# C0ldstudy/PointSecGuard

Measured on AMD Instinct MI355X. Metric: attacked rooms/sec (4096 pts, 40 PGD iters), higher is better.
Workload: dtype f32; 1 GPU; NB non-targeted PGD (eps=0.05, alpha=2/255, 40 iters) on PointNet++ SSG sem_seg, batch=8 rooms x 4096 pts x 9 ch per GPU (BASELINE configs[1]); steps_coalesced_per_launch_max=8, device_batch_rooms=64, launches_in_flight_per_gpu=3, weights=tests/golden/pn2_weights.npz (fitted fixture)

## Files before the change

include/psg.h:

```cpp
#ifndef PSG_H
#define PSG_H

#include <stdint.h>

#ifdef __cplusplus
extern "C" {
#endif

#define PSG_OK 0
#define PSG_ERR_ARG (-1)
#define PSG_ERR_HIP (-2)
#define PSG_ERR_STATE (-3)

typedef struct psg_ctx psg_ctx;
typedef struct psg_pn2_model psg_pn2_model;
typedef struct psg_pn2_ws psg_pn2_ws;
typedef void *psg_stream;

const char *psg_last_error(void);
const char *psg_version(void);
int psg_env_switches(char *buf, int cap);
int psg_diag_build(void);

int psg_ctx_create(int device, psg_ctx **out);
// ... 46 lines not shown
int psg_pn2_forward(psg_pn2_model *model, psg_pn2_ws *ws, int forward, const float *x0, float *logp_out,
                    float *l4_out, psg_stream stream);

int psg_pn2_backward(psg_pn2_model *model, psg_pn2_ws *ws, int forward, const float *dlogp, float *dx0_out,
                     psg_stream stream);
int psg_pn2_backward_full(psg_pn2_model *model, psg_pn2_ws *ws, int forward, const float *dlogp, float *dx0_out,
                          psg_stream stream);

int psg_pn2_forward_lean(psg_pn2_model *model, psg_pn2_ws *ws, int forward, const float *x0, float *logp_out,
                         psg_stream stream);
int psg_pn2_backward_colour(psg_pn2_model *model, psg_pn2_ws *ws, int forward, const float *dlogp, float *dx0_out,
                            psg_stream stream);
int psg_pn2_backward_colour_pgd(psg_pn2_model *model, psg_pn2_ws *ws, int forward, const float *dlogp, float *x,
                                const float *ori, const uint8_t *mask, float alpha, float eps, float dir, int last,
                                psg_stream stream);

const float *psg_pn2_activation_ptr(const psg_pn2_ws *ws, int which);
int psg_pn2_activation_channels(const psg_pn2_ws *ws, int which);


int psg_group_rows(const float *xyz, const float *feat, const float *new_xyz, const int32_t *gidx, int B, int N, int S,
                   int K, int D, int feat_first, float *rows_out, psg_stream stream);
int psg_group_rows_bwd(const float *drows, const int32_t *gidx, int B, int N, int S, int K, int D, int feat_first,
                       float *dfeat, psg_stream stream);
int psg_pw_mlp_fwd(const float *in, int ld_in, int rows, int K, const float *w, const float *bias, int relu, int M,
                   float *out, int ld_out, uint32_t *mask_out, const float *scale, const float *shift, psg_stream stream);
int psg_pw_mlp_bwd(const float *dout, int ld_dout, int rows, int M, const float *wT, const uint32_t *mask_below, int K,
                   float *din, int ld_din, psg_stream stream);
int psg_apply_relu_bits(float *g, int ld, const uint32_t *bits, const float *scale, int rows, int M, psg_stream stream);
int psg_sa_mlp_max_fwd(const float *rows_in, int n_groups, int K, int cin, int n_layers, const int *widths,
// ... 570 lines not shown
```

pointsecguard_amd/_lib.py:

```python
import ctypes
import os

_HERE = os.path.dirname(os.path.abspath(__file__))
LIB_PATH = os.environ.get("PSG_LIBRARY_OVERRIDE") or os.path.join(_HERE, "libpsg.so")

c_f = ctypes.POINTER(ctypes.c_float)
c_i = ctypes.POINTER(ctypes.c_int32)
c_u8 = ctypes.POINTER(ctypes.c_uint8)
c_ll = ctypes.POINTER(ctypes.c_longlong)
vp = ctypes.c_void_p
ci = ctypes.c_int
cf = ctypes.c_float

SIGNATURES = {
    "psg_last_error": (ctypes.c_char_p, []),
    "psg_version": (ctypes.c_char_p, []),
    "psg_env_switches": (ci, [ctypes.c_char_p, ci]),
    "psg_diag_build": (ci, []),
    "psg_ctx_create": (ci, [ci, ctypes.POINTER(vp)]),
    "psg_ctx_destroy": (ci, [vp]),
    "psg_square_distance": (ci, [vp, vp, vp, ci, ci, ci, vp, vp]),
    "psg_fps": (ci, [vp, vp, ci, ci, ci, ci, vp, vp, vp]),
    "psg_gather_points": (ci, [vp, vp, ci, ci, ci, ci, vp, ci, vp, vp]),
    "psg_ball_query": (ci, [vp, vp, ci, vp, ci, ci, ci, cf, ci, vp, vp]),
# ... 20 lines not shown
    "psg_pn2_ws_create": (ci, [vp, ci, ci, ci, ctypes.POINTER(vp)]),
    "psg_pn2_ws_create_arch": (ci, [vp, ci, ci, ci, ci, ctypes.POINTER(vp)]),
    "psg_pn2_ws_destroy": (ci, [vp]),
    "psg_pn2_ws_bytes": (ctypes.c_size_t, [vp]),
    "psg_pn2_debug_read": (ci, [vp, ctypes.POINTER(ctypes.c_ulonglong), ci]),
    "psg_pn2_prof_enable": (ci, [vp, ci]),
    "psg_pn2_prof_read": (ci, [vp, ci, ctypes.POINTER(ctypes.c_double), ctypes.POINTER(ctypes.c_int)]),
    "psg_pn2_plan_build": (ci, [vp, vp, vp, ci, vp]),
    "psg_pn2_plan_ptr": (vp, [vp, ci, ci, ci, ci]),
    "psg_pn2_forward": (ci, [vp, vp, ci, vp, vp, vp, vp]),
    "psg_pn2_backward": (ci, [vp, vp, ci, vp, vp, vp]),
    "psg_pn2_backward_full": (ci, [vp, vp, ci, vp, vp, vp]),
    "psg_pn2_forward_lean": (ci, [vp, vp, ci, vp, vp, vp]),
    "psg_pn2_backward_colour": (ci, [vp, vp, ci, vp, vp, vp]),
    "psg_pn2_backward_colour_pgd": (ci, [vp, vp, ci, vp, vp, vp, vp, cf, cf, cf, ci, vp]),
    "psg_pn2_activation_ptr": (vp, [vp, ci]),
    "psg_pn2_activation_channels": (ci, [vp, ci]),
    "psg_to_point_major": (ci, [vp, ci, ci, ci, vp, vp]),
    "psg_to_channel_major": (ci, [vp, ci, ci, ci, vp, vp]),
    "psg_ce_logp_grad": (ci, [vp, vp, ci, ci, ci, ci, cf, vp, vp, vp]),
    "psg_pgd_step": (ci, [vp, vp, vp, vp, ci, ci, cf, cf, cf, ci, vp]),
    "psg_pgd_step_field": (ci, [vp, vp, vp, vp, ci, ci, ci, cf, cf, cf, ci, vp]),
    "psg_pn2_nb_attack": (ci, [vp, vp, vp, vp, vp, vp, cf, cf, ci, ci, ci, vp, vp]),
    "psg_pointnet_model_create": (ci, [vp, ctypes.POINTER(vp), ctypes.POINTER(vp), ctypes.POINTER(vp)]),
    "psg_pointnet_model_destroy": (ci, [vp]),
    "psg_pointnet_ws_create": (ci, [vp, ci, ci, ctypes.POINTER(vp)]),
    "psg_pointnet_ws_destroy": (ci, [vp]),
    "psg_pointnet_forward": (ci, [vp, vp, vp, vp, vp, vp, vp, vp, vp]),
    "psg_pointnet_backward": (ci, [vp, vp, vp, vp, vp, vp]),
    "psg_pointnet_nb_attack": (ci, [vp, vp, vp, vp, vp, cf, cf, ci, ci, ci, vp, vp]),
# ... 259 lines not shown
```

pointsecguard_amd/csrc/psg_api.hip:

```cpp
#include <mutex>
#include <atomic>
#include <stdarg.h>
#include <stdlib.h>
#include <string.h>
#include <unordered_set>

#include "psg_common.h"

namespace {
thread_local char g_err[512] = "";
}

namespace psg {
struct EnvSwitch { const char *name; char kind; };
static const EnvSwitch kEnvSwitches[] = {
    {"PSG_TRACE_SYNC", 'd'},       {"PSG_GCN_KNN_STATS", 'd'},   {"PSG_KNN_XCD_ORDER", 'p'},  {"PSG_KNN_FINE_CUT_KK", 'p'},  {"PSG_KNN_SAMPLE2_KK", 'p'},  {"PSG_KNN_F32_SAMPLED_KK", 'p'},
    {"PSG_FP1_WAVE", 'p'},         {"PSG_RLA_NO_FUSE16", 'p'},   {"PSG_RLA_ATOMICS", 'p'},    {"PSG_RLA_NO_SPLIT", 'p'},
    {"PSG_RLA_NO_GRAPH", 'p'},     {"PSG_GEMM_SMALL_BELOW", 'p'}, {"PSG_GCN_KNN", 'p'},        {"PSG_GCN_KNN_BF_MAXD", 'p'},
    {"PSG_GCN_PQ_FUSION", 'p'},    {"PSG_GCN_NO_GRAPH", 'p'},    {"PSG_GCN_EDGE_BWD", 'p'},   {"PSG_BALL_QUERY", 'p'},
    {"PSG_PN2_SPLIT", 'p'},          {"PSG_RLA_NO_DIRECT", 'p'},   {"PSG_NU_NO_GRAPH", 'p'},      {"PSG_PN2_GRAPH", 'p'},
    {"PSG_PN2_FPSPLIT", 'p'},        {"PSG_FPS_CFG", 'p'},         {"PSG_PN2_L1T_COLOUR", 'p'},
    {"PSG_PN2_PGD_FUSE", 'p'},       {"PSG_PN2_POOLT_SPARSE", 'p'}, {"PSG_PN2_PW_SIZED", 'p'},
    {"PSG_PN2_BALL_TABLE", 'p'},     {"PSG_PN2_PACK", 'p'},          {"PSG_PN2_PACK_BWD", 'p'},
    {"PSG_PN2_POOLT_ORDER", 'p'},    {"PSG_THREE_NN", 'p'},
#ifdef PSG_DIAG_BUILD
    {"PSG_DIAG", 'r'},
#endif
};

hipError_t copy_sync(void *dst, const void *src, size_t bytes, hipMemcpyKind kind)
{
    if (bytes == 0) return hipSuccess;
    hipStream_t st = nullptr;
    hipError_t e = hipStreamCreateWithFlags(&st, hipStreamNonBlocking);
    if (e != hipSuccess) return e;
    e = hipMemcpyAsync(dst, src, bytes, kind, st);
    if (e == hipSuccess) e = hipStreamSynchronize(st);
    (void)hipStreamDestroy(st);
    return e;
// ... 185 lines not shown
```

pointsecguard_amd/csrc/psg_attack.hip:

```cpp
#include <string.h>

#include "psg_adam.cuh"
#include "psg_common.h"

namespace {

__global__ void to_point_major_kernel(const float *__restrict__ src, float *__restrict__ dst, int C, int N, size_t total)
{
    for (size_t t = (size_t)blockIdx.x * blockDim.x + threadIdx.x; t < total; t += (size_t)gridDim.x * blockDim.x) {
        size_t b = t / N, n = t % N;
        for (int c = 0; c < C; ++c) dst[t * C + c] = src[(b * C + c) * N + n];
    }
}

__global__ void to_channel_major_kernel(const float *__restrict__ src, float *__restrict__ dst, int C, int N,
                                        size_t total)
{
    for (size_t t = (size_t)blockIdx.x * blockDim.x + threadIdx.x; t < total; t += (size_t)gridDim.x * blockDim.x) {
        size_t b = t / N, n = t % N;
        for (int c = 0; c < C; ++c) dst[(b * C + c) * N + n] = src[t * C + c];
    }
}

constexpr int MAXC = 32;

__global__ __launch_bounds__(256) void ce_logp_grad_kernel(const float *__restrict__ logp, const int32_t *__restrict__ labels, int target,
                                                            int rows, int rows_active, int n_cls, float scale, float *__restrict__ dlogp,
                                                            float *__restrict__ cost)
{
    __shared__ float s_z[256 * MAXC];
    const int r0 = blockIdx.x * 256, nr = min(256, rows - r0);
    const float *src = logp + (size_t)r0 * n_cls;
    for (int i = threadIdx.x; i < nr * n_cls; i += 256) s_z[i] = src[i];
    __syncthreads();
    const int r = r0 + (int)threadIdx.x;
    float g[MAXC];
    if ((int)threadIdx.x < nr) {
        if (r >= rows_active) {
            for (int c = 0; c < n_cls; ++c) g[c] = 0.0f;
        } else {
            const float *lp = s_z + threadIdx.x * n_cls;
            float z[MAXC];
            float m = -INFINITY;
            for (int c = 0; c < n_cls; ++c) { z[c] = lp[c]; m = fmaxf(m, z[c]); }
            float s = 0.0f;
            for (int c = 0; c < n_cls; ++c) s += expf(z[c] - m);
            const float lse = logf(s);
            const int y = labels ? labels[r] : target;
            for (int c = 0; c < n_cls; ++c) {
                float lp2 = (z[c] - m) - lse;
                float p = expf(lp2);
                g[c] = (p - (c == y ? 1.0f : 0.0f)) * scale;
                if (cost && c == y) atomicAdd(cost, -lp2 * scale);
            }
        }
    }
    __syncthreads();
    if ((int)threadIdx.x < nr) {
        float *o = s_z + threadIdx.x * n_cls;
        for (int c = 0; c < n_cls; ++c) o[c] = g[c];
    }
    __syncthreads();
    float *dst = dlogp + (size_t)r0 * n_cls;
    for (int i = threadIdx.x; i < nr * n_cls; i += 256) dst[i] = s_z[i];
}

__global__ void pgd_step_kernel(float *__restrict__ x, const float *__restrict__ grad, const float *__restrict__ ori,
                                const uint8_t *__restrict__ mask, int N, size_t total, float step, float eps, int last)
{
    for (size_t t = (size_t)blockIdx.x * blockDim.x + threadIdx.x; t < total * 3; t += (size_t)gridDim.x * blockDim.x) {
// ... 1002 lines not shown
```

pointsecguard_amd/csrc/psg_pn2.hip:

```cpp
#include <algorithm>
#include <cstdlib>
#include <cstring>
#include <vector>

#include "psg_common.h"
#include "psg_pn2_kernels.cuh"
#include "psg_chain.cuh"
#include "psg_pn2_geomgrad.cuh"

using namespace psg;

namespace {

constexpr int MAXL = PSG_PN2_MSG_NUM_LAYERS;
constexpr int NCLS = PSG_PN2_NUM_CLASSES;
const int kS[4] = {1024, 256, 64, 16};

static inline int diag_build_bits()
{
#ifdef PSG_DIAG_BUILD
    static const int bits = psg::env_int("PSG_DIAG", 0);
    return bits;
#else
    return 0;
// ... 279 lines not shown
FwdLayer fwd_layer(const PackedLayer &p, bool relu, uint16_t *mask)
{
    FwdLayer f;
    f.w = p.wf; f.bias = p.bias; f.mask = mask; f.k8 = p.k8f(); f.mb = p.mbf(); f.relu = relu ? 1 : 0;
    return f;
}
BwdLayer bwd_layer(const PackedLayer &p, const uint16_t *mask)
{
    BwdLayer f;
    f.w = p.wb; f.mask = mask; f.k8 = p.k8b(); f.mb = p.mbb();
    return f;
}

enum { TAG_SA_FWD = 0, TAG_FP_FWD = 4, TAG_FP_BWD = 8, TAG_SA_BWD = 12, TAG_FPS = 16, TAG_BALL = 17, TAG_NN = 18,
       TAG_GATHER = 19, TAG_CE = 20, TAG_PGD = 21, TAG_ZERO = 22, TAG_PW_FWD = 23, TAG_PW_BWD = 24,
       TAG_GEOM_GREL = 25, TAG_GEOM_WGRAD = 26, TAG_GEOM_GX = 27, TAG_PACK_PLAN = 28, TAG_COUNT = 29 };

template <typename KernelT, typename ArgsT>
int launch_lds(psg_pn2_ws *ws, int tag, const char *site, KernelT kern, dim3 grid, int threads, int blocks8, int blk,
               const ArgsT &args, hipStream_t st)
{
    size_t lds = (size_t)blocks8 * blk * sizeof(float);
    if (lds > 160 * 1024) { set_error("LDS request %zu exceeds 160 KiB", lds); return PSG_ERR_ARG; }
    if (lds > 48 * 1024) PSG_CHECK_HIP(psg::allow_big_lds((const void *)kern));
    EvScope prof(&ws->prof, tag, 0.0, st);
    hipLaunchKernelGGL(kern, grid, dim3(threads), lds, st, args);
    PSG_LAUNCH_CHECK_AT(site);
    return PSG_OK;
}

inline int layer_blocks(int k8, int mb) { return std::max(k8, mb * 4); }
// ... 574 lines not shown
int run_fp_fwd(psg_pn2_model *m, psg_pn2_ws *ws, int fwd, float *logp, hipStream_t st)
{
    if constexpr (FpCfg<LVL>::P2 != FpCfg<LVL>::P)
        if (ws->Nl[LVL] % FpCfg<LVL>::P2 == 0) return run_fp_fwd_p<LVL, FpCfg<LVL>::P2>(m, ws, fwd, logp, st);
    return run_fp_fwd_p<LVL, FpCfg<LVL>::P>(m, ws, fwd, logp, st);
}

template <int LVL>
int run_fp_bwd(psg_pn2_model *m, psg_pn2_ws *ws, int fwd, const float *logp, const float *dlogp, hipStream_t st)
{
    if constexpr (FpCfg<LVL>::P2 != FpCfg<LVL>::P)
        if (ws->Nl[LVL] % FpCfg<LVL>::P2 == 0) return run_fp_bwd_p<LVL, FpCfg<LVL>::P2>(m, ws, fwd, logp, dlogp, st);
    return run_fp_bwd_p<LVL, FpCfg<LVL>::P>(m, ws, fwd, logp, dlogp, st);
}

__global__ void extract_xyz_kernel(const float *__restrict__ x0, float *__restrict__ xyz, size_t rows)
{
    for (size_t t = (size_t)blockIdx.x * blockDim.x + threadIdx.x; t < rows * 3; t += (size_t)gridDim.x * blockDim.x)
        xyz[t] = x0[(t / 3) * 9 + (t % 3)];
}

__global__ void extract_color_kernel(const float *__restrict__ x0, float *__restrict__ ori, size_t rows)
{
    for (size_t t = (size_t)blockIdx.x * blockDim.x + threadIdx.x; t < rows * 3; t += (size_t)gridDim.x * blockDim.x)
        ori[t] = x0[(t / 3) * 9 + 3 + (t % 3)];
}

__global__ void gather_starts_kernel(const int32_t *__restrict__ starts, int32_t *__restrict__ out, int level, int B,
                                     int P)
{
// ... 630 lines not shown
    }
}

extern "C" const float *psg_pn2_activation_ptr(const psg_pn2_ws *ws, int which)
{
    if (!ws || which < 0 || which > 6) return nullptr;
    return ws->act[which];
}

extern "C" int psg_pn2_activation_channels(const psg_pn2_ws *ws, int which)
{
    if (!ws || which < 0 || which > 6) return 0;
    return ws->actC[which];
}

extern "C" int psg_pn2_forward(psg_pn2_model *m, psg_pn2_ws *ws, int fwd, const float *x0, float *logp_out,
                               float *l4_out, psg_stream stream)
{
    PSG_REQUIRE(m && ws && x0 && logp_out, "psg_pn2_forward: null argument");
    PSG_REQUIRE(m->arch == ws->arch, "psg_pn2_forward: model and workspace were created for different architectures");
    PSG_REQUIRE(fwd >= 0 && fwd < ws->planned, "psg_pn2_forward: plan slot %d not built (planned %d)", fwd, ws->planned);
    hipStream_t st = (hipStream_t)stream;
    int rc;
    ws->x0_fwd = x0;
    for (int l = 0; l < 4; ++l) {
        for (int sc = 0; sc < m->arch->ns; ++sc) {
            if (m->split_fwd[l] && (rc = run_pw_fwd(m, ws, l, sc, fwd, st))) return rc;
            if ((rc = run_sa_fwd(m, ws, l, sc, fwd, x0, st))) return rc;
        }
    }
    if ((rc = run_fp_fwd<3>(m, ws, fwd, nullptr, st))) return rc;
    if ((rc = run_fp_fwd<2>(m, ws, fwd, nullptr, st))) return rc;
    if ((rc = run_fp_fwd<1>(m, ws, fwd, nullptr, st))) return rc;
    if ((rc = run_fp_fwd<0>(m, ws, fwd, ws->logp, st))) return rc;
    if (logp_out != ws->logp)
        PSG_CHECK_HIP(hipMemcpyAsync(logp_out, ws->logp, (size_t)ws->B * ws->N * NCLS * 4, hipMemcpyDeviceToDevice, st));
    if (l4_out)
        PSG_CHECK_HIP(hipMemcpyAsync(l4_out, ws->act[3], (size_t)ws->B * 16 * ws->actC[3] * 4, hipMemcpyDeviceToDevice, st));
    ws->fwd_slot = fwd;
    return PSG_OK;
}

static int backward_impl(psg_pn2_model *m, psg_pn2_ws *ws, int fwd, const float *logp, const float *dlogp,
                         float *dx0, int c_lo, int c_hi, hipStream_t st, const PgdFuse *pgd = nullptr, bool rel0 = false)
{
    const ArchDesc &A = *m->arch;
    int rc;
    if ((rc = run_fp_bwd<0>(m, ws, fwd, logp, dlogp, st))) return rc;
    if ((rc = run_fp_bwd<1>(m, ws, fwd, nullptr, nullptr, st))) return rc;
    if ((rc = run_fp_bwd<2>(m, ws, fwd, nullptr, nullptr, st))) return rc;
    if ((rc = run_fp_bwd<3>(m, ws, fwd, nullptr, nullptr, st))) return rc;
    for (int l = 3; l >= 0; --l) {
        for (int sc = 0; sc < A.ns; ++sc) {
            if ((rc = run_sa_bwd(m, ws, l, sc, fwd, l ? 0 : c_lo, l ? A.C[l] : (rel0 ? A.C[0] + 3 : c_hi), st))) return rc;
            if (m->split[l] && (rc = run_pw_bwd(m, ws, l, sc, fwd, st))) return rc;
        }
    }
    {
        EvScope prof(&ws->prof, TAG_ZERO, 0.0, st);
        const bool compact = c_hi - c_lo == 3;
        const size_t total = (size_t)ws->B * ws->N * (compact ? 1 : c_hi - c_lo);
        const dim3 grid((unsigned)std::min<size_t>(8192, (total + 255) / 256));
        const size_t po = (size_t)fwd * ws->B * (ws->N + 1);
// ... 154 lines not shown
}
extern "C" int psg_pn2_backward_colour(psg_pn2_model *m, psg_pn2_ws *ws, int fwd, const float *dlogp, float *dx0_out, psg_stream stream)
{
    return psg::pn2_backward_colour(m, ws, fwd, dlogp, dx0_out, stream);
}
extern "C" int psg_pn2_backward_colour_pgd(psg_pn2_model *m, psg_pn2_ws *ws, int fwd, const float *dlogp, float *x, const float *ori,
                                           const uint8_t *mask, float alpha, float eps, float dir, int last, psg_stream stream)
{
    PSG_REQUIRE(m && ws && dlogp && x && ori, "psg_pn2_backward_colour_pgd: null argument");
    PSG_REQUIRE(dir == 1.0f || dir == -1.0f, "psg_pn2_backward_colour_pgd: dir must be +1 or -1");
    if (int rc = require_resident(m, ws, fwd, "psg_pn2_backward_colour_pgd")) return rc;
    const PgdFuse pf{x, ori, mask, dir * alpha, eps, last ? 1 : 0};
    return backward_impl(m, ws, fwd, ws->logp, dlogp, ws->dx0, 3, 6, (hipStream_t)stream, &pf);
}

extern "C" int psg_pn2_nb_attack(psg_pn2_model *m, psg_pn2_ws *ws, const float *images, const int32_t *labels,
                                 const int32_t *starts, const uint8_t *mask, float eps, float alpha, int iters,
                                 int targeted, int target, float *adv_out, psg_stream stream)
{
    PSG_REQUIRE(m && ws && images && starts && adv_out, "psg_pn2_nb_attack: null argument");
    PSG_REQUIRE(m->arch == ws->arch, "psg_pn2_nb_attack: model and workspace were created for different architectures");
    PSG_REQUIRE(targeted || labels, "psg_pn2_nb_attack: labels required for the non-targeted attack");
    PSG_REQUIRE(iters > 0 && iters <= ws->F, "psg_pn2_nb_attack: iters=%d exceeds workspace capacity %d", iters, ws->F);
    hipStream_t st = (hipStream_t)stream;
    const int B = ws->B, N = ws->N;
    int rc;
    if ((rc = psg_to_point_major(images, B, 9, N, ws->x0, st))) return rc;
    if (!targeted) PSG_CHECK_HIP(hipMemcpyAsync(ws->nb_labels, labels, (size_t)B * N * sizeof(int32_t), hipMemcpyDeviceToDevice, st));
    PSG_CHECK_HIP(hipMemcpyAsync(ws->nb_starts, starts, (size_t)iters * 4 * B * sizeof(int32_t), hipMemcpyDeviceToDevice, st));
    if (mask) PSG_CHECK_HIP(hipMemcpyAsync(ws->nb_mask, mask, (size_t)N, hipMemcpyDeviceToDevice, st));
    const int32_t *labels_ws = targeted ? nullptr : ws->nb_labels;
    const uint8_t *mask_ws = mask ? ws->nb_mask : nullptr;
    auto body = [&](hipStream_t st) -> int {
        int r;
        hipLaunchKernelGGL(extract_color_kernel, dim3(std::min(1024, ceil_div(B * N * 3, 256))), dim3(256), 0, st, ws->x0,
                           ws->ori, (size_t)B * N);
        PSG_LAUNCH_CHECK();
        if ((r = psg_pn2_plan_build(ws, ws->x0, ws->nb_starts, iters, st))) return r;
        const int rows = B * N;
        for (int it = 0; it < iters; ++it) {
            if ((r = psg::pn2_forward_lean(m, ws, it, ws->x0, ws->logp, st))) return r;
            {
                EvScope prof(&ws->prof, TAG_CE, 0.0, st);
                if ((r = psg_ce_logp_grad(ws->logp, labels_ws, target, rows, targeted ? N : rows, NCLS, 1.0f / (float)N, ws->dlogp,
                                          nullptr, st)))
                    return r;
            }
            static const bool pgd_fuse = psg::env_int("PSG_PN2_PGD_FUSE", 1) != 0;
            if (pgd_fuse) {
                const PgdFuse pf{ws->x0, ws->ori, mask_ws, (targeted ? -1.0f : 1.0f) * alpha, eps, it == iters - 1 ? 1 : 0};
                if ((r = backward_impl(m, ws, it, ws->logp, ws->dlogp, ws->dx0, 3, 6, st, &pf))) return r;
            } else {
                if ((r = backward_impl(m, ws, it, ws->logp, ws->dlogp, ws->dx0, 3, 6, st))) return r;
                EvScope prof(&ws->prof, TAG_PGD, 0.0, st);
                if ((r = psg_pgd_step(ws->x0, ws->dx0, ws->ori, mask_ws, B, N, alpha, eps, targeted ? -1.0f : 1.0f, it == iters - 1, st)))
                    return r;
            }
        }
        return PSG_OK;
    };
    static const bool use_graph = psg::env_int("PSG_PN2_GRAPH", 0) != 0 && !psg::trace_sync_enabled();
    if (use_graph && B <= 16 && !ws->prof.on) {
        const psg_pn2_ws::NbKey key{m->gen, eps, alpha, iters, targeted ? 1 : 0, targeted ? target : 0, mask ? 1 : 0, targeted ? 0 : 1, 0};
        const bool same = ws->nb_have_key && memcmp(&key, &ws->nb_key, sizeof(key)) == 0;
        if (same && !ws->nb.capture_failed) {
            if (!ws->nb_stream) {
                PSG_CHECK_HIP(hipStreamCreateWithFlags(&ws->nb_stream, hipStreamNonBlocking));
                for (hipEvent_t &e : ws->nb_ev) PSG_CHECK_HIP(hipEventCreateWithFlags(&e, hipEventDisableTiming));
            }
            hipStream_t gs = ws->nb_stream;
            PSG_CHECK_HIP(hipEventRecord(ws->nb_ev[0], st));
            PSG_CHECK_HIP(hipStreamWaitEvent(gs, ws->nb_ev[0], 0));
            if (ws->nb.exec || ws->nb.capture(gs, [&] { return body(gs); })) {
                PSG_CHECK_HIP(ws->nb.replay(gs));
                ws->planned = iters; ws->fwd_slot = iters - 1; ws->x0_fwd = ws->x0;
                PSG_CHECK_HIP(hipEventRecord(ws->nb_ev[1], gs));
                PSG_CHECK_HIP(hipStreamWaitEvent(st, ws->nb_ev[1], 0));
                return psg_to_channel_major(ws->x0, B, 9, N, adv_out, st);
            }
        }
        if (!same) {
            PSG_CHECK_HIP(ws->nb.forget(st));
            ws->nb_key = key;
            ws->nb_have_key = true;
        }
        ws->nb.note_eager();
    }
    if ((rc = body(st))) return rc;
    return psg_to_channel_major(ws->x0, B, 9, N, adv_out, st);
}
// ... 1 lines not shown
```

pointsecguard_amd/csrc/psg_pn2_kernels.cuh:

```cuda
#pragma once
#include "psg_mlp.cuh"

#ifdef PSG_DIAG_BUILD
#define PSG_DIAGBIT(a, bit) ((a).diag & (bit))
#else
#define PSG_DIAGBIT(a, bit) 0
#endif

namespace psg {

struct SaFwdArgs {
    const float *xyz;
    const float *feat;
    const float *new_xyz;
    const int32_t *gidx;
    float *out;
    uint8_t *arg;
    FwdLayer l1, l2;
    const float4 *w3;
    const float *b3;
    int k8_3, nb3;
    int xyz_stride, D, Np, S, C3;
    int ld_out, c_out;
    const float *tfeat;
// ... 1752 lines not shown
    for (int j = rg; j < P; j += RG) {
        const unsigned o = __umul24((unsigned)j, (unsigned)w2);
        for (int q = ql; q < (w2 >> 2); q += 32) *(float4 *)(d2 + (o + 4u * q)) = *(const float4 *)(in + L::off(o2 + 4 * q, j));
    }
    if (!d1) return;
    if (a.split) {
        layer_bwd<P, NW, MAXT>(a.skipT, in, wg);
        __syncthreads();
    }
    for (int j = rg; j < P; j += RG) {
        const unsigned o = __umul24((unsigned)j, (unsigned)a.C1);
        for (int q = ql; q < (a.C1 >> 2); q += 32) *(float4 *)(d1 + (o + 4u * q)) = *(const float4 *)(in + L::off(4 * q, j));
    }
}

struct PwBwdArgs {
    const int32_t *ginv_off;
    const float *gsa;
    int g_rows;
    const float *skip;
    float *out;
    BwdLayer wt;
    int N, C1, D;
};

template <int P, int NW, int VW>
__device__ __forceinline__ void pw_bwd_gather_rows(const PwBwdArgs &a, int b, int n0, float *__restrict__ buf, int lane, int wave)
{
    static_assert(P == 32, "one 32-point tile per workgroup");
    typedef float vwf __attribute__((ext_vector_type(VW)));
// ... 129 lines not shown
```

pointsecguard_amd/runtime.py:

```python
import ctypes

import numpy as np
import torch

from . import _lib

SA_NPOINT = (1024, 256, 64, 16)
SA_RADIUS = (0.1, 0.2, 0.4, 0.8)
NSAMPLE = 32
SA_PACK_GROUPS = (4, 2, 1, 1)
SA_WIDTH3 = (64, 128, 256, 512)
NUM_CLASSES = 13
ARCH_SSG, ARCH_MSG = 0, 1
ARCH_LAYERS = {ARCH_SSG: 23, ARCH_MSG: 35}
MSG_NSAMPLE = (16, 32)
ACT_POINTS = (1024, 256, 64, 16, 64, 256, 1024)
ACT_SHAPES = ((1024, 64), (256, 128), (64, 256), (16, 512), (64, 256), (256, 256), (1024, 128))

_ctx = {}
_hip = None


def ptr(t):
    if t is None:
# ... 192 lines not shown
        out = torch.empty_like(images)
        _lib.call("psg_to_channel_major", ptr(x0), B, 9, N, ptr(out), stream())
        return out

    def backward_pgd(self, model, slot, dlogp, x0, ori, alpha, eps, mask=None, descent=False, last=False):
        require_cuda(dlogp, "dlogp", torch.float32)
        require_cuda(x0, "x0", torch.float32)
        require_cuda(ori, "ori", torch.float32)
        if mask is not None:
            require_cuda(mask, "mask", torch.uint8)
        assert x0.shape == (self.batch, self.n_point, 9) and ori.shape == (self.batch, self.n_point, 3) and x0.is_contiguous() and ori.is_contiguous()
        _lib.call("psg_pn2_backward_colour_pgd", model.handle, self.handle, slot, ptr(dlogp), ptr(x0), ptr(ori), ptr(mask),
                  float(alpha), float(eps), -1.0 if descent else 1.0, 1 if last else 0, stream())
        return x0

    def nb_attack(self, model, images, labels, starts, eps, alpha, iters, mask=None, target=None, out=None):
        require_cuda(images, "images", torch.float32)
        require_cuda(starts, "starts", torch.int32)
        if labels is not None:
            require_cuda(labels, "labels", torch.int32)
        if mask is not None:
            require_cuda(mask, "mask", torch.uint8)
        if out is None:
            out = torch.empty_like(images)
        _lib.call("psg_pn2_nb_attack", model.handle, self.handle, ptr(images), ptr(labels), ptr(starts), ptr(mask),
                  float(eps), float(alpha), int(iters), 0 if target is None else 1, 0 if target is None else int(target),
                  ptr(out), stream())
        return out

    PROF_TAGS = ("sa1_fwd", "sa2_fwd", "sa3_fwd", "sa4_fwd", "fp1_head_fwd", "fp2_fwd", "fp3_fwd", "fp4_fwd",
                 "fp1_head_bwd", "fp2_bwd", "fp3_bwd", "fp4_bwd", "sa1_bwd", "sa2_bwd", "sa3_bwd", "sa4_bwd",
                 "fps", "ball_query", "three_nn", "gather", "ce_grad", "pgd_step", "dx0_gather", "pw_fwd", "pw_bwd",
                 "geom_grel", "geom_wgrad", "geom_gx", "sa_pack_plan")

    def prof_enable(self, on=True):
        _lib.call("psg_pn2_prof_enable", self.handle, 1 if on else 0)

    def prof_read(self):
        n = len(self.PROF_TAGS)
        ms = (ctypes.c_double * n)()
        cnt = (ctypes.c_int * n)()
        _lib.call("psg_pn2_prof_read", self.handle, n, ms, cnt)
        return {t: (ms[i], cnt[i]) for i, t in enumerate(self.PROF_TAGS) if cnt[i]}

    def plan_tensor(self, what, level, forward, room):
        n_l = (self.n_point,) + SA_NPOINT
        k0 = MSG_NSAMPLE[0] if self.arch == ARCH_MSG else NSAMPLE
        shape, dt = {0: ((SA_NPOINT[level],), torch.int32), 1: ((SA_NPOINT[level], k0), torch.int32),
# ... 448 lines not shown
```

Before: 1042 rooms/s.

## Fuse FP1 head forward, cross-entropy grad and FP1 backward into one kernel

Adds a single fp1_loop_kernel that runs the FP1 layers and classifier head forward, computes log-softmax and the cross-entropy gradient in LDS, then runs the FP1/head backward chain in the same workgroup, writing only the gradient into FP2. The PGD attack loop is refactored into an nb_step that takes this path when the model shape matches, skipping the separate FP1 forward, CE kernel and FP1 backward launches along with their global-memory round trips for activations, logp and dlogp. The CE row math is shared through a new header. The cost is a complex, shape-specialised kernel with heavy LDS and register use, and a gate that falls back to the old path when the layer configuration differs.

```diff
diff --git a/include/psg.h b/include/psg.h
--- a/include/psg.h
+++ b/include/psg.h
@@ -84,6 +84,10 @@
 int psg_pn2_backward_colour_pgd(psg_pn2_model *model, psg_pn2_ws *ws, int forward, const float *dlogp, float *x,
                                 const float *ori, const uint8_t *mask, float alpha, float eps, float dir, int last,
                                 psg_stream stream);
+
+int psg_pn2_nb_step(psg_pn2_model *model, psg_pn2_ws *ws, int forward, float *x, const float *ori, const int32_t *labels,
+                    const uint8_t *mask, float alpha, float eps, int targeted, int target, int last, psg_stream stream);
+const float *psg_pn2_fp1_grad_ptr(const psg_pn2_ws *ws);
 
 const float *psg_pn2_activation_ptr(const psg_pn2_ws *ws, int which);
 int psg_pn2_activation_channels(const psg_pn2_ws *ws, int which);
diff --git a/pointsecguard_amd/_lib.py b/pointsecguard_amd/_lib.py
--- a/pointsecguard_amd/_lib.py
+++ b/pointsecguard_amd/_lib.py
@@ -58,6 +58,8 @@
     "psg_pn2_forward_lean": (ci, [vp, vp, ci, vp, vp, vp]),
     "psg_pn2_backward_colour": (ci, [vp, vp, ci, vp, vp, vp]),
     "psg_pn2_backward_colour_pgd": (ci, [vp, vp, ci, vp, vp, vp, vp, cf, cf, cf, ci, vp]),
+    "psg_pn2_nb_step": (ci, [vp, vp, ci, vp, vp, vp, vp, cf, cf, ci, ci, ci, vp]),
+    "psg_pn2_fp1_grad_ptr": (vp, [vp]),
     "psg_pn2_activation_ptr": (vp, [vp, ci]),
     "psg_pn2_activation_channels": (ci, [vp, ci]),
     "psg_to_point_major": (ci, [vp, ci, ci, ci, vp, vp]),
diff --git a/pointsecguard_amd/csrc/psg_api.hip b/pointsecguard_amd/csrc/psg_api.hip
--- a/pointsecguard_amd/csrc/psg_api.hip
+++ b/pointsecguard_amd/csrc/psg_api.hip
@@ -22,7 +22,7 @@
     {"PSG_PN2_FPSPLIT", 'p'},        {"PSG_FPS_CFG", 'p'},         {"PSG_PN2_L1T_COLOUR", 'p'},
     {"PSG_PN2_PGD_FUSE", 'p'},       {"PSG_PN2_POOLT_SPARSE", 'p'}, {"PSG_PN2_PW_SIZED", 'p'},
     {"PSG_PN2_BALL_TABLE", 'p'},     {"PSG_PN2_PACK", 'p'},          {"PSG_PN2_PACK_BWD", 'p'},
-    {"PSG_PN2_POOLT_ORDER", 'p'},    {"PSG_THREE_NN", 'p'},
+    {"PSG_PN2_POOLT_ORDER", 'p'},    {"PSG_THREE_NN", 'p'},         {"PSG_PN2_FP1_LOOP", 'p'},
 #ifdef PSG_DIAG_BUILD
     {"PSG_DIAG", 'r'},
 #endif
diff --git a/pointsecguard_amd/csrc/psg_attack.hip b/pointsecguard_amd/csrc/psg_attack.hip
--- a/pointsecguard_amd/csrc/psg_attack.hip
+++ b/pointsecguard_amd/csrc/psg_attack.hip
@@ -1,6 +1,7 @@
 #include <string.h>
 
 #include "psg_adam.cuh"
+#include "psg_ce_row.cuh"
 #include "psg_common.h"
 
 namespace {
@@ -22,7 +23,7 @@
     }
 }
 
-constexpr int MAXC = 32;
+constexpr int MAXC = psg::CE_ROW_MAXC;
 
 __global__ __launch_bounds__(256) void ce_logp_grad_kernel(const float *__restrict__ logp, const int32_t *__restrict__ labels, int target,
                                                             int rows, int rows_active, int n_cls, float scale, float *__restrict__ dlogp,
@@ -36,24 +37,10 @@
     const int r = r0 + (int)threadIdx.x;
     float g[MAXC];
     if ((int)threadIdx.x < nr) {
-        if (r >= rows_active) {
-            for (int c = 0; c < n_cls; ++c) g[c] = 0.0f;
-        } else {
-            const float *lp = s_z + threadIdx.x * n_cls;
-            float z[MAXC];
-            float m = -INFINITY;
-            for (int c = 0; c < n_cls; ++c) { z[c] = lp[c]; m = fmaxf(m, z[c]); }
-            float s = 0.0f;
-            for (int c = 0; c < n_cls; ++c) s += expf(z[c] - m);
-            const float lse = logf(s);
-            const int y = labels ? labels[r] : target;
-            for (int c = 0; c < n_cls; ++c) {
-                float lp2 = (z[c] - m) - lse;
-                float p = expf(lp2);
-                g[c] = (p - (c == y ? 1.0f : 0.0f)) * scale;
-                if (cost && c == y) atomicAdd(cost, -lp2 * scale);
-            }
-        }
+        const bool active = r < rows_active;
+        const int y = !active ? -1 : labels ? labels[r] : target;
+        const float term = psg::ce_row_grad(s_z + threadIdx.x * n_cls, n_cls, y, scale, active, g);
+        if (cost && active && y >= 0 && y < n_cls) atomicAdd(cost, term);
     }
     __syncthreads();
     if ((int)threadIdx.x < nr) {
diff --git a/pointsecguard_amd/csrc/psg_ce_row.cuh b/pointsecguard_amd/csrc/psg_ce_row.cuh
--- /dev/null
+++ b/pointsecguard_amd/csrc/psg_ce_row.cuh
@@ -0,0 +1,37 @@
+#pragma once
+#include <math.h>
+
+#if defined(__HIPCC__) || defined(__CUDACC__)
+#define PSG_CE_ROW_FN __host__ __device__ __forceinline__
+#else
+#define PSG_CE_ROW_FN inline
+#endif
+
+namespace psg {
+
+constexpr int CE_ROW_MAXC = 32;
+
+PSG_CE_ROW_FN float ce_row_grad(const float *lp, int n_cls, int y, float scale, bool active, float *g)
+{
+#pragma clang fp contract(off)
+    if (!active) {
+        for (int c = 0; c < n_cls; ++c) g[c] = 0.0f;
+        return 0.0f;
+    }
+    float z[CE_ROW_MAXC];
+    float m = -INFINITY;
+    for (int c = 0; c < n_cls; ++c) { z[c] = lp[c]; m = fmaxf(m, z[c]); }
+    float s = 0.0f;
+    for (int c = 0; c < n_cls; ++c) s += __builtin_expf(z[c] - m);
+    const float lse = __builtin_logf(s);
+    float term = 0.0f;
+    for (int c = 0; c < n_cls; ++c) {
+        const float lp2 = (z[c] - m) - lse;
+        const float p = __builtin_expf(lp2);
+        g[c] = (p - (c == y ? 1.0f : 0.0f)) * scale;
+        if (c == y) term = -lp2 * scale;
+    }
+    return term;
+}
+
+}
diff --git a/pointsecguard_amd/csrc/psg_pn2.hip b/pointsecguard_amd/csrc/psg_pn2.hip
--- a/pointsecguard_amd/csrc/psg_pn2.hip
+++ b/pointsecguard_amd/csrc/psg_pn2.hip
@@ -317,7 +317,8 @@
 
 enum { TAG_SA_FWD = 0, TAG_FP_FWD = 4, TAG_FP_BWD = 8, TAG_SA_BWD = 12, TAG_FPS = 16, TAG_BALL = 17, TAG_NN = 18,
        TAG_GATHER = 19, TAG_CE = 20, TAG_PGD = 21, TAG_ZERO = 22, TAG_PW_FWD = 23, TAG_PW_BWD = 24,
-       TAG_GEOM_GREL = 25, TAG_GEOM_WGRAD = 26, TAG_GEOM_GX = 27, TAG_PACK_PLAN = 28, TAG_COUNT = 29 };
+       TAG_GEOM_GREL = 25, TAG_GEOM_WGRAD = 26, TAG_GEOM_GX = 27, TAG_PACK_PLAN = 28, TAG_FP1_LOOP = 29,
+       TAG_COUNT = 30 };
 
 template <typename KernelT, typename ArgsT>
 int launch_lds(psg_pn2_ws *ws, int tag, const char *site, KernelT kern, dim3 grid, int threads, int blocks8, int blk,
@@ -922,6 +923,57 @@
     return run_fp_bwd_p<LVL, FpCfg<LVL>::P>(m, ws, fwd, logp, dlogp, st);
 }
 
+bool fp1_loop_applies(const psg_pn2_model *m, const psg_pn2_ws *ws)
+{
+    static const bool on = psg::env_int("PSG_PN2_FP1_LOOP", 1) != 0;
+#ifdef PSG_DIAG_BUILD
+    constexpr bool diag_build = true;
+#else
+    constexpr bool diag_build = false;
+#endif
+    if (!on || diag_build || FpCfg<0>::P2 != 64 || FpCfg<0>::NW != 4 || fp1_wave() || !m->fsplit[0] || ws->Nl[0] % 64) return false;
+    const ArchDesc &A = *m->arch;
+    const int first = A.fp_first[0], head = A.head;
+    if (A.fp_count[0] != 3 || NCLS != 13 || m->fa[0].k8f() != 0 || m->fa[0].cout != 128 || m->fb[0].cout != 128) return false;
+    for (const PackedLayer *p : {&m->L[first + 1], &m->L[first + 2], &m->L[head]})
+        if (p->k8f() != 16 || p->mbf() != 4 || p->k8b() != 16 || p->mbb() != 4) return false;
+    const PackedLayer &c2 = m->L[head + 1];
+    return c2.k8f() == 16 && c2.mbf() == 1 && c2.k8b() == 2 && c2.mbb() == 4;
+}
+
+int run_fp1_loop(psg_pn2_model *m, psg_pn2_ws *ws, int fwd, const int32_t *labels, int target, int rows_active, float scale,
+                 hipStream_t st)
+{
+    constexpr int P = 64, NW = 4;
+    const ArchDesc &A = *m->arch;
+    const int B = ws->B, N = ws->Nl[0], first = A.fp_first[0], head = A.head;
+    const size_t prob = (size_t)fwd * B;
+    Fp1LoopArgs a{};
+    a.fwd.nn_idx = ws->nn_idx[0] + prob * N * 3;
+    a.fwd.nn_w = ws->nn_w[0] + prob * N * 3;
+    a.fwd.tsrc = ws->tfp[0]; a.fwd.ldt = m->fa[0].cout;
+    a.fwd.N = N; a.fwd.S = ws->Nl[1];
+    a.fwd.layer[0] = fwd_layer(m->fa[0], true, nullptr);
+    a.fwd.layer[0].bias = m->L[first].bias;
+    a.f[0] = fwd_layer(m->L[first + 1], true, nullptr);
+    a.f[1] = fwd_layer(m->L[first + 2], true, nullptr);
+    a.f[2] = fwd_layer(m->L[head], true, nullptr);
+    a.head = fwd_layer(m->L[head + 1], false, nullptr);
+    a.t[0] = bwd_layer(m->L[head + 1], nullptr);
+    a.t[1] = bwd_layer(m->L[head], nullptr);
+    a.t[2] = bwd_layer(m->L[first + 2], nullptr);
+    a.t[3] = bwd_layer(m->L[first + 1], nullptr);
+    a.labels = labels; a.target = target; a.rows_active = rows_active; a.scale = scale;
+    a.dint_out = ws->dint[0];
+    a.N = N;
+#if PSG_MLP_PAIRS
+    return launch_lds(ws, TAG_FP1_LOOP, PSG_SITE, (fp1_loop_kernel<P, NW, NCLS>), dim3(N / P, B), NW * 64, 16 + PSG_LDS_SPARE, Lds<P>::BLK, a, st);
+#else
+    set_error("run_fp1_loop: built without the paired k-loop");
+    return PSG_ERR_STATE;
+#endif
+}
+
 __global__ void extract_xyz_kernel(const float *__restrict__ x0, float *__restrict__ xyz, size_t rows)
 {
     for (size_t t = (size_t)blockIdx.x * blockDim.x + threadIdx.x; t < rows * 3; t += (size_t)gridDim.x * blockDim.x)
@@ -1582,13 +1634,8 @@
     return ws->actC[which];
 }
 
-extern "C" int psg_pn2_forward(psg_pn2_model *m, psg_pn2_ws *ws, int fwd, const float *x0, float *logp_out,
-                               float *l4_out, psg_stream stream)
-{
-    PSG_REQUIRE(m && ws && x0 && logp_out, "psg_pn2_forward: null argument");
-    PSG_REQUIRE(m->arch == ws->arch, "psg_pn2_forward: model and workspace were created for different architectures");
-    PSG_REQUIRE(fwd >= 0 && fwd < ws->planned, "psg_pn2_forward: plan slot %d not built (planned %d)", fwd, ws->planned);
-    hipStream_t st = (hipStream_t)stream;
+static int forward_to_fp2(psg_pn2_model *m, psg_pn2_ws *ws, int fwd, const float *x0, hipStream_t st)
+{
     int rc;
     ws->x0_fwd = x0;
     for (int l = 0; l < 4; ++l) {
@@ -1599,7 +1646,18 @@
     }
     if ((rc = run_fp_fwd<3>(m, ws, fwd, nullptr, st))) return rc;
     if ((rc = run_fp_fwd<2>(m, ws, fwd, nullptr, st))) return rc;
-    if ((rc = run_fp_fwd<1>(m, ws, fwd, nullptr, st))) return rc;
+    return run_fp_fwd<1>(m, ws, fwd, nullptr, st);
+}
+
+extern "C" int psg_pn2_forward(psg_pn2_model *m, psg_pn2_ws *ws, int fwd, const float *x0, float *logp_out,
+                               float *l4_out, psg_stream stream)
+{
+    PSG_REQUIRE(m && ws && x0 && logp_out, "psg_pn2_forward: null argument");
+    PSG_REQUIRE(m->arch == ws->arch, "psg_pn2_forward: model and workspace were created for different architectures");
+    PSG_REQUIRE(fwd >= 0 && fwd < ws->planned, "psg_pn2_forward: plan slot %d not built (planned %d)", fwd, ws->planned);
+    hipStream_t st = (hipStream_t)stream;
+    int rc;
+    if ((rc = forward_to_fp2(m, ws, fwd, x0, st))) return rc;
     if ((rc = run_fp_fwd<0>(m, ws, fwd, ws->logp, st))) return rc;
     if (logp_out != ws->logp)
         PSG_CHECK_HIP(hipMemcpyAsync(logp_out, ws->logp, (size_t)ws->B * ws->N * NCLS * 4, hipMemcpyDeviceToDevice, st));
@@ -1610,11 +1668,12 @@
 }
 
 static int backward_impl(psg_pn2_model *m, psg_pn2_ws *ws, int fwd, const float *logp, const float *dlogp,
-                         float *dx0, int c_lo, int c_hi, hipStream_t st, const PgdFuse *pgd = nullptr, bool rel0 = false)
+                         float *dx0, int c_lo, int c_hi, hipStream_t st, const PgdFuse *pgd = nullptr, bool rel0 = false,
+                         bool fp1_done = false)
 {
     const ArchDesc &A = *m->arch;
     int rc;
-    if ((rc = run_fp_bwd<0>(m, ws, fwd, logp, dlogp, st))) return rc;
+    if (!fp1_done && (rc = run_fp_bwd<0>(m, ws, fwd, logp, dlogp, st))) return rc;
     if ((rc = run_fp_bwd<1>(m, ws, fwd, nullptr, nullptr, st))) return rc;
     if ((rc = run_fp_bwd<2>(m, ws, fwd, nullptr, nullptr, st))) return rc;
     if ((rc = run_fp_bwd<3>(m, ws, fwd, nullptr, nullptr, st))) return rc;
@@ -1799,6 +1858,53 @@
     return backward_impl(m, ws, fwd, ws->logp, dlogp, ws->dx0, 3, 6, (hipStream_t)stream, &pf);
 }
 
+static int nb_step(psg_pn2_model *m, psg_pn2_ws *ws, int fwd, float *x, const float *ori, const int32_t *labels, const uint8_t *mask,
+                   float alpha, float eps, int targeted, int target, bool last, hipStream_t st)
+{
+    const int B = ws->B, N = ws->N, rows = B * N;
+    const int rows_active = targeted ? N : rows;
+    const float scale = 1.0f / (float)N, dir = targeted ? -1.0f : 1.0f;
+    const bool fused = fp1_loop_applies(m, ws);
+    int r;
+    if (fused) {
+        PSG_REQUIRE(fwd >= 0 && fwd < ws->planned, "psg_pn2_nb_step: plan slot %d not built (planned %d)", fwd, ws->planned);
+        ws->lean = true;
+        r = forward_to_fp2(m, ws, fwd, x, st);
+        ws->lean = false;
+        ws->fwd_slot = -1;
+        if (r) return r;
+        if ((r = run_fp1_loop(m, ws, fwd, labels, target, rows_active, scale, st))) return r;
+    } else {
+        if ((r = psg::pn2_forward_lean(m, ws, fwd, x, ws->logp, st))) return r;
+        EvScope prof(&ws->prof, TAG_CE, 0.0, st);
+        if ((r = psg_ce_logp_grad(ws->logp, labels, target, rows, rows_active, NCLS, scale, ws->dlogp, nullptr, st))) return r;
+    }
+    static const bool pgd_fuse = psg::env_int("PSG_PN2_PGD_FUSE", 1) != 0;
+    if (pgd_fuse) {
+        const PgdFuse pf{x, ori, mask, dir * alpha, eps, last ? 1 : 0};
+        return backward_impl(m, ws, fwd, ws->logp, ws->dlogp, ws->dx0, 3, 6, st, &pf, false, fused);
+    }
+    if ((r = backward_impl(m, ws, fwd, ws->logp, ws->dlogp, ws->dx0, 3, 6, st, nullptr, false, fused))) return r;
+    EvScope prof(&ws->prof, TAG_PGD, 0.0, st);
+    return psg_pgd_step(x, ws->dx0, ori, mask, B, N, alpha, eps, dir, last, st);
+}
+
+extern "C" int psg_pn2_nb_step(psg_pn2_model *m, psg_pn2_ws *ws, int fwd, float *x, const float *ori, const int32_t *labels,
+                               const uint8_t *mask, float alpha, float eps, int targeted, int target, int last, psg_stream stream)
+{
+    PSG_REQUIRE(m && ws && x && ori, "psg_pn2_nb_step: null argument");
+    PSG_REQUIRE(m->arch == ws->arch, "psg_pn2_nb_step: model and workspace were created for different architectures");
+    PSG_REQUIRE(targeted || labels, "psg_pn2_nb_step: labels required for the non-targeted step");
+    PSG_REQUIRE(!targeted || (target >= 0 && target < NCLS), "psg_pn2_nb_step: target class %d out of range", target);
+    PSG_REQUIRE(fwd >= 0 && fwd < ws->planned, "psg_pn2_nb_step: plan slot %d not built (planned %d)", fwd, ws->planned);
+    return nb_step(m, ws, fwd, x, ori, targeted ? nullptr : labels, mask, alpha, eps, targeted, target, last != 0, (hipStream_t)stream);
+}
+
+extern "C" const float *psg_pn2_fp1_grad_ptr(const psg_pn2_ws *ws)
+{
+    return ws ? ws->dint[0] : nullptr;
+}
+
 extern "C" int psg_pn2_nb_attack(psg_pn2_model *m, psg_pn2_ws *ws, const float *images, const int32_t *labels,
                                  const int32_t *starts, const uint8_t *mask, float eps, float alpha, int iters,
                                  int targeted, int target, float *adv_out, psg_stream stream)
@@ -1822,26 +1928,8 @@
                            ws->ori, (size_t)B * N);
         PSG_LAUNCH_CHECK();
         if ((r = psg_pn2_plan_build(ws, ws->x0, ws->nb_starts, iters, st))) return r;
-        const int rows = B * N;
-        for (int it = 0; it < iters; ++it) {
-            if ((r = psg::pn2_forward_lean(m, ws, it, ws->x0, ws->logp, st))) return r;
-            {
-                EvScope prof(&ws->prof, TAG_CE, 0.0, st);
-                if ((r = psg_ce_logp_grad(ws->logp, labels_ws, target, rows, targeted ? N : rows, NCLS, 1.0f / (float)N, ws->dlogp,
-                                          nullptr, st)))
-                    return r;
-            }
-            static const bool pgd_fuse = psg::env_int("PSG_PN2_PGD_FUSE", 1) != 0;
-            if (pgd_fuse) {
-                const PgdFuse pf{ws->x0, ws->ori, mask_ws, (targeted ? -1.0f : 1.0f) * alpha, eps, it == iters - 1 ? 1 : 0};
-                if ((r = backward_impl(m, ws, it, ws->logp, ws->dlogp, ws->dx0, 3, 6, st, &pf))) return r;
-            } else {
-                if ((r = backward_impl(m, ws, it, ws->logp, ws->dlogp, ws->dx0, 3, 6, st))) return r;
-                EvScope prof(&ws->prof, TAG_PGD, 0.0, st);
-                if ((r = psg_pgd_step(ws->x0, ws->dx0, ws->ori, mask_ws, B, N, alpha, eps, targeted ? -1.0f : 1.0f, it == iters - 1, st)))
-                    return r;
-            }
-        }
+        for (int it = 0; it < iters; ++it)
+            if ((r = nb_step(m, ws, it, ws->x0, ws->ori, labels_ws, mask_ws, alpha, eps, targeted, target, it == iters - 1, st))) return r;
         return PSG_OK;
     };
     static const bool use_graph = psg::env_int("PSG_PN2_GRAPH", 0) != 0 && !psg::trace_sync_enabled();
@@ -1858,7 +1946,7 @@
             PSG_CHECK_HIP(hipStreamWaitEvent(gs, ws->nb_ev[0], 0));
             if (ws->nb.exec || ws->nb.capture(gs, [&] { return body(gs); })) {
                 PSG_CHECK_HIP(ws->nb.replay(gs));
-                ws->planned = iters; ws->fwd_slot = iters - 1; ws->x0_fwd = ws->x0;
+                ws->planned = iters; ws->fwd_slot = fp1_loop_applies(m, ws) ? -1 : iters - 1; ws->x0_fwd = ws->x0;
                 PSG_CHECK_HIP(hipEventRecord(ws->nb_ev[1], gs));
                 PSG_CHECK_HIP(hipStreamWaitEvent(st, ws->nb_ev[1], 0));
                 return psg_to_channel_major(ws->x0, B, 9, N, adv_out, st);
diff --git a/pointsecguard_amd/csrc/psg_pn2_kernels.cuh b/pointsecguard_amd/csrc/psg_pn2_kernels.cuh
--- a/pointsecguard_amd/csrc/psg_pn2_kernels.cuh
+++ b/pointsecguard_amd/csrc/psg_pn2_kernels.cuh
@@ -1,4 +1,5 @@
 #pragma once
+#include "psg_ce_row.cuh"
 #include "psg_mlp.cuh"
 
 #ifdef PSG_DIAG_BUILD
@@ -1790,6 +1791,181 @@
     }
 }
 
+struct Fp1LoopArgs {
+    FpFwdArgs fwd;
+    FwdLayer f[3];
+    FwdLayer head;
+    BwdLayer t[4];
+    const int32_t *labels;
+    int target, rows_active;
+    float scale;
+    float *dint_out;
+    int N;
+};
+
+__device__ __forceinline__ void add_bias16(f32x16 &c, const float4 &bq0, const float4 &bq1, const float4 &bq2, const float4 &bq3)
+{
+    c[0] += bq0.x; c[1] += bq0.y; c[2] += bq0.z; c[3] += bq0.w;
+    c[4] += bq1.x; c[5] += bq1.y; c[6] += bq1.z; c[7] += bq1.w;
+    c[8] += bq2.x; c[9] += bq2.y; c[10] += bq2.z; c[11] += bq2.w;
+    c[12] += bq3.x; c[13] += bq3.y; c[14] += bq3.z; c[15] += bq3.w;
+}
+
+template <int P>
+__device__ __forceinline__ unsigned fp1_loop_pair_bits(const float *__restrict__ buf, int first, int lane)
+{
+    const int j = lane & 31, h = lane >> 5;
+    const float *o = buf + (size_t)(first * 4) * Lds<P>::BLK + j * 8 + 4 * h;
+    unsigned m = 0;
+#pragma unroll
+    for (int pb = 0; pb < 2; ++pb) {
+#pragma unroll
+        for (int g = 0; g < 4; ++g) {
+            const float4 v = *(const float4 *)(o + (size_t)g * Lds<P>::BLK + pb * 32 * 8);
+            m |= (v.x > 0.0f ? 1u : 0u) << (16 * pb + 4 * g);
+            m |= (v.y > 0.0f ? 1u : 0u) << (16 * pb + 4 * g + 1);
+            m |= (v.z > 0.0f ? 1u : 0u) << (16 * pb + 4 * g + 2);
+            m |= (v.w > 0.0f ? 1u : 0u) << (16 * pb + 4 * g + 3);
+        }
+    }
+    return m;
+}
+
+template <int P>
+__device__ __forceinline__ unsigned fp1_loop_pair_fwd(const FwdLayer &Lr, float *__restrict__ buf, int first, int lane)
+{
+    constexpr int BLK = Lds<P>::BLK;
+    const int j = lane & 31, h = lane >> 5;
+    const float4 *bp = (const float4 *)(Lr.bias + first * 32 + 4 * h);
+    const float4 bq0 = bp[0], bq1 = bp[2], bq2 = bp[4], bq3 = bp[6];
+    f32x16 c0, c1;
+#pragma unroll
+    for (int r = 0; r < 16; ++r) { c0[r] = 0.0f; c1[r] = 0.0f; }
+    tile_mac_x2<BLK, false>(Lr.w + (size_t)first * Lr.k8 * 64 + lane, Lr.k8, buf + j * 8 + 4 * h, c0, c1);
+    add_bias16(c0, bq0, bq1, bq2, bq3);
+    const unsigned m0 = relu_bits(c0);
+    add_bias16(c1, bq0, bq1, bq2, bq3);
+    const unsigned m1 = relu_bits(c1);
+    __syncthreads();
+    store_tile<P>(buf, first, j, h, c0);
+    store_tile<P>(buf, first, 32 + j, h, c1);
+    return m0 | (m1 << 16);
+}
+
+template <int P>
+__device__ __forceinline__ void fp1_loop_pair_bwd(const BwdLayer &Lt, float *__restrict__ buf, int first, int lane, unsigned m)
+{
+    constexpr int BLK = Lds<P>::BLK;
+    const int j = lane & 31, h = lane >> 5;
+    f32x16 c0, c1;
+#pragma unroll
+    for (int r = 0; r < 16; ++r) { c0[r] = 0.0f; c1[r] = 0.0f; }
+    tile_mac_x2<BLK, false>(Lt.w + (size_t)first * Lt.k8 * 64 + lane, Lt.k8, buf + j * 8 + 4 * h, c0, c1);
+    apply_bits(c0, m);
+    apply_bits(c1, m >> 16);
+    __syncthreads();
+    store_tile<P>(buf, first, j, h, c0);
+    store_tile<P>(buf, first, 32 + j, h, c1);
+}
+
+template <int P, int NW, int NC>
+__global__ __launch_bounds__(NW * 64) __attribute__((amdgpu_waves_per_eu(4))) void fp1_loop_kernel(Fp1LoopArgs a)
+{
+    static_assert(P == 64 && NW == 4 && NC <= 16, "one pair of tiles per wave and 128-wide layer; the classes in two LDS blocks");
+    using L = Lds<P>;
+    constexpr int NT = NW * 64;
+    extern __shared__ float lds[];
+    float *buf0 = lds;
+    const int tid = threadIdx.x, lane = tid & 63, wave = tid >> 6;
+    const int j = lane & 31, h = lane >> 5;
+    int bx, b;
+    xcd_tile(bx, b);
+    const int n0 = bx * P;
+    const size_t wg = (size_t)b * gridDim.x + bx;
+    const int first = (wave + (int)(wg & (NW - 1))) & (NW - 1);
+
+    fp_layer1_split<P, NW>(a.fwd, b, n0, buf0, wg);
+    __syncthreads();
+    const unsigned m_l1 = fp1_loop_pair_bits<P>(buf0, first, lane);
+    const unsigned m_l2 = fp1_loop_pair_fwd<P>(a.f[0], buf0, first, lane);
+    __syncthreads();
+    const unsigned m_l3 = fp1_loop_pair_fwd<P>(a.f[1], buf0, first, lane);
+    __syncthreads();
+    const unsigned m_c1 = fp1_loop_pair_fwd<P>(a.f[2], buf0, first, lane);
+    __syncthreads();
+    {
+        f32x16 c;
+        if (first < P / 32) {
+            const float4 *bp = (const float4 *)(a.head.bias + 4 * h);
+            const float4 bq0 = bp[0], bq1 = bp[2], bq2 = bp[4], bq3 = bp[6];
+#pragma unroll
+            for (int r = 0; r < 16; ++r) c[r] = 0.0f;
+            c = tile_mac<L::BLK, false>(a.head.w + lane, a.head.k8, buf0 + (first * 32 + j) * 8 + 4 * h, c);
+            add_bias16(c, bq0, bq1, bq2, bq3);
+        }
+        __syncthreads();
+        if (first < P / 32) store_tile<P>(buf0, 0, first * 32 + j, h, c);
+    }
+    __syncthreads();
+
+    float *s_lp = buf0 + (size_t)4 * L::BLK, *s_dl = buf0 + (size_t)6 * L::BLK;
+    for (int t = tid; t < P * 8; t += NT) {
+        const int pj = t >> 3, q = t & 7;
+        const bool has0 = q < NC;
+        const float z0 = has0 ? buf0[L::off(q, pj)] : -INFINITY;
+        const bool has1 = q + 8 < NC;
+        const float z1 = has1 ? buf0[L::off(q + 8, pj)] : -INFINITY;
+        float m = fmaxf(z0, z1);
+        m = fmaxf(m, __shfl_xor(m, 1));
+        m = fmaxf(m, __shfl_xor(m, 2));
+        m = fmaxf(m, __shfl_xor(m, 4));
+        float s = (has0 ? expf(z0 - m) : 0.0f) + (has1 ? expf(z1 - m) : 0.0f);
+        s += __shfl_xor(s, 1);
+        s += __shfl_xor(s, 2);
+        s += __shfl_xor(s, 4);
+        const float lse = logf(s);
+        float *o = s_lp + pj * NC;
+        if (has0) o[q] = (z0 - m) - lse;
+        if (has1) o[q + 8] = (z1 - m) - lse;
+    }
+    __syncthreads();
+    if (tid < P) {
+        const int r = b * a.N + n0 + tid;
+        const bool active = r < a.rows_active;
+        const int y = !active ? -1 : a.labels ? a.labels[r] : a.target;
+        ce_row_grad(s_lp + tid * NC, NC, y, a.scale, active, s_dl + tid * NC);
+    }
+    __syncthreads();
+    for (int t = tid; t < P * 4; t += NT) {
+        const int pj = t >> 2, q = t & 3;
+        const float *lp = s_lp + pj * NC, *dl = s_dl + pj * NC;
+        float s = 0.0f;
+        if (q == 0)
+            for (int c = 0; c < NC; ++c) s += dl[c];
+        s = __shfl(s, (tid & 63) & ~3);
+#pragma unroll
+        for (int i = 0; i < 4; ++i) {
+            const int c = q + 4 * i;
+            buf0[L::off(c, pj)] = c < NC ? dl[c] - expf(lp[c]) * s : 0.0f;
+        }
+    }
+    __syncthreads();
+
+    fp1_loop_pair_bwd<P>(a.t[0], buf0, first, lane, m_c1);
+    __syncthreads();
+    fp1_loop_pair_bwd<P>(a.t[1], buf0, first, lane, m_l3);
+    __syncthreads();
+    fp1_loop_pair_bwd<P>(a.t[2], buf0, first, lane, m_l2);
+    __syncthreads();
+    fp1_loop_pair_bwd<P>(a.t[3], buf0, first, lane, m_l1);
+    __syncthreads();
+    constexpr int RG = NT / 32, CD = 128;
+    const int ql = tid & 31, rg = tid >> 5;
+    float *d2 = a.dint_out + ((size_t)b * a.N + n0) * CD;
+    for (int pj = rg; pj < P; pj += RG)
+        *(float4 *)(d2 + (pj * CD + 4 * ql)) = *(const float4 *)(buf0 + L::off(4 * ql, pj));
+}
+
 struct PwBwdArgs {
     const int32_t *ginv_off;
     const float *gsa;
diff --git a/pointsecguard_amd/runtime.py b/pointsecguard_amd/runtime.py
--- a/pointsecguard_amd/runtime.py
+++ b/pointsecguard_amd/runtime.py
@@ -230,6 +230,24 @@
                   float(alpha), float(eps), -1.0 if descent else 1.0, 1 if last else 0, stream())
         return x0
 
+    def nb_step(self, model, slot, x0, ori, labels, alpha, eps, mask=None, target=None, last=False):
+        require_cuda(x0, "x0", torch.float32)
+        require_cuda(ori, "ori", torch.float32)
+        if labels is not None:
+            require_cuda(labels, "labels", torch.int32)
+        if mask is not None:
+            require_cuda(mask, "mask", torch.uint8)
+        assert x0.shape == (self.batch, self.n_point, 9) and ori.shape == (self.batch, self.n_point, 3) and x0.is_contiguous() and ori.is_contiguous()
+        _lib.call("psg_pn2_nb_step", model.handle, self.handle, slot, ptr(x0), ptr(ori), ptr(labels), ptr(mask), float(alpha),
+                  float(eps), 0 if target is None else 1, 0 if target is None else int(target), 1 if last else 0, stream())
+        return x0
+
+    def fp1_grad(self):
+        src = _lib.load().psg_pn2_fp1_grad_ptr(self.handle)
+        out = torch.empty(self.batch, self.n_point, 128, dtype=torch.float32, device=self.device)
+        _hip_memcpy_d2d(out.data_ptr(), src, out.numel() * 4)
+        return out
+
     def nb_attack(self, model, images, labels, starts, eps, alpha, iters, mask=None, target=None, out=None):
         require_cuda(images, "images", torch.float32)
         require_cuda(starts, "starts", torch.int32)
@@ -247,7 +265,7 @@
     PROF_TAGS = ("sa1_fwd", "sa2_fwd", "sa3_fwd", "sa4_fwd", "fp1_head_fwd", "fp2_fwd", "fp3_fwd", "fp4_fwd",
                  "fp1_head_bwd", "fp2_bwd", "fp3_bwd", "fp4_bwd", "sa1_bwd", "sa2_bwd", "sa3_bwd", "sa4_bwd",
                  "fps", "ball_query", "three_nn", "gather", "ce_grad", "pgd_step", "dx0_gather", "pw_fwd", "pw_bwd",
-                 "geom_grel", "geom_wgrad", "geom_gx", "sa_pack_plan")
+                 "geom_grel", "geom_wgrad", "geom_gx", "sa_pack_plan", "fp1_head_loop")
 
     def prof_enable(self, on=True):
         _lib.call("psg_pn2_prof_enable", self.handle, 1 if on else 0)
```

New measurement: 1055 rooms/s (median of 6 runs). 1.01x the previous value.
